# SiftScience/kafka-assigner

Hardware: NVIDIA H100
Metric: partition-replica assignments/sec (higher is better)
Workload: dtype int32

## Files before the change

### kafka_assigner_b200/csrc/kassign_common.cuh

```cuda
#pragma once
#include <cuda_runtime.h>
#include <stdint.h>

#define KA_MAX_SLOTS 8
#define KA_DEAD 0xFFFFu
#define KA_FULL 0xFFFFFFFFu

#define KA_E_RF_MISMATCH 1
#define KA_E_RF_NOT_POSITIVE 2
#define KA_E_RF_GT_BROKERS 3
#define KA_E_UNASSIGNABLE 4
#define KA_E_HASH_INDEX 5

enum { KA_LUT_SMEM = 0, KA_LUT_GLOBAL = 1, KA_LUT_BSEARCH = 2 };

struct KaBrokers {
    int N, lut_mode, lut_off, blob_bytes, min_id;
    uint32_t range;
    const uint16_t* blob;
    const uint16_t* glut;
    const int32_t* broker_id;
};

struct KaStageOut {
    unsigned char* rec;
    uint16_t* perm;
    int32_t* ntl;
    uint32_t* lend;
    int4* tstatus;
    unsigned* err_topic;
};

struct KaCandidate {
    KaBrokers br;
    KaStageOut out;
    int32_t* ctr8;
    const int32_t* loff;
    uint32_t pos0;
    int t0, T;
    uint32_t row0, Q;
    int desired_rf;
};

__device__ __forceinline__ uint32_t ka_lookup(int id, const uint16_t* lut, const KaBrokers& br) {
    if (br.lut_mode == KA_LUT_SMEM) {
        uint32_t off = (uint32_t)id - (uint32_t)br.min_id;
        return off < br.range ? (uint32_t)lut[off] : KA_DEAD;
    } else if (br.lut_mode == KA_LUT_GLOBAL) {
        uint32_t off = (uint32_t)id - (uint32_t)br.min_id;
        return off < br.range ? (uint32_t)__ldg(&br.glut[off]) : KA_DEAD;
    } else {
        int lo = 0, hi = br.N - 1;
        while (lo <= hi) {
            int mid = (lo + hi) >> 1;
            int v = __ldg(&br.broker_id[mid]);
            if (v == id) return (uint32_t)mid;
            if (v < id) lo = mid + 1; else hi = mid - 1;
        }
        return KA_DEAD;
    }
}



__device__ __forceinline__ uint32_t ka_smem_u32(const void* p) { return (uint32_t)__cvta_generic_to_shared(p); }

__device__ __forceinline__ void ka_mbar_init(uint64_t* bar, uint32_t count) {
    asm volatile("mbarrier.init.shared::cta.b64 [%0], %1;" ::"r"(ka_smem_u32(bar)), "r"(count));
}
__device__ __forceinline__ void ka_fence_mbar_init() { asm volatile("fence.mbarrier_init.release.cluster;" ::: "memory"); }
__device__ __forceinline__ void ka_fence_proxy_async() { asm volatile("fence.proxy.async.shared::cta;" ::: "memory"); }
__device__ __forceinline__ void ka_mbar_expect_tx(uint64_t* bar, uint32_t bytes) {
    asm volatile("mbarrier.arrive.expect_tx.shared::cta.b64 _, [%0], %1;" ::"r"(ka_smem_u32(bar)), "r"(bytes) : "memory");
}
__device__ __forceinline__ void ka_mbar_wait(uint64_t* bar, uint32_t parity) {
    asm volatile(
        "{\n"
        ".reg .pred p;\n"
        "WAIT_LOOP:\n"
        "mbarrier.try_wait.parity.shared::cta.b64 p, [%0], %1;\n"
        "@p bra WAIT_DONE;\n"
        "bra WAIT_LOOP;\n"
        "WAIT_DONE:\n"
        "}\n" ::"r"(ka_smem_u32(bar)),
        "r"(parity)
        : "memory");
}
__device__ __forceinline__ void ka_tma_bulk_g2s(void* dst_smem, const void* src_gmem, uint32_t bytes, uint64_t* bar) {
    asm volatile("cp.async.bulk.shared::cluster.global.mbarrier::complete_tx::bytes [%0], [%1], %2, [%3];" ::"r"(
                     ka_smem_u32(dst_smem)),
                 "l"(src_gmem), "r"(bytes), "r"(ka_smem_u32(bar))
                 : "memory");
}

__device__ __forceinline__ int4 ka_ldg_stream_v4(const int4* p) {
    int4 r;
    asm volatile("ld.global.nc.L1::no_allocate.v4.s32 {%0,%1,%2,%3}, [%4];" : "=r"(r.x), "=r"(r.y), "=r"(r.z), "=r"(r.w) : "l"(p));
    return r;
}

__device__ __forceinline__ uint32_t ka_lanemask_lt() {
    uint32_t m;
    asm("mov.u32 %0, %%lanemask_lt;" : "=r"(m));
    return m;
}

__device__ __forceinline__ uint32_t ka_rot_bits(uint32_t habs) {
    return ((habs % 2u) << 4) | ((habs % 3u) << 5) | ((habs % 4u) << 7) | ((habs % 5u) << 9) | ((habs % 6u) << 12) |
           ((habs % 7u) << 15) | ((habs % 8u) << 18);
}
template <int RS>
__device__ __forceinline__ int ka_rot_of(uint32_t meta, int k) {
    int s = 0;
    if (k == 2) s = (meta >> 4) & 1u;
    if (k == 3) s = (meta >> 5) & 3u;
    if (k == 4) s = (meta >> 7) & 3u;
    if (RS > 4) {
        if (k == 5) s = (meta >> 9) & 7u;
        if (k == 6) s = (meta >> 12) & 7u;
        if (k == 7) s = (meta >> 15) & 7u;
        if (k == 8) s = (meta >> 18) & 7u;
    }
    return s;
}
```

### kafka_assigner_b200/csrc/kassign_order.cuh

```cuda
#pragma once
#include "kassign_common.cuh"

__global__ void __launch_bounds__(1024) ka_level_scan_kernel(const int32_t* __restrict__ ntl, int T, int32_t* __restrict__ loff) {
    __shared__ int wsum[32];
    __shared__ int carry;
    const int lane = threadIdx.x & 31, warp = threadIdx.x >> 5;
    if (threadIdx.x == 0) carry = 0;
    __syncthreads();
    for (int t0 = 0; t0 < T; t0 += 1024) {
        const int t = t0 + threadIdx.x;
        const int v = t < T ? ntl[t] : 0;
        int x = v;
#pragma unroll
        for (int o = 1; o < 32; o <<= 1) {
            const int y = __shfl_up_sync(KA_FULL, x, o);
            if (lane >= o) x += y;
        }
        if (lane == 31) wsum[warp] = x;
        __syncthreads();
        if (warp == 0) {
            int w = wsum[lane];
#pragma unroll
            for (int o = 1; o < 32; o <<= 1) {
                const int y = __shfl_up_sync(KA_FULL, w, o);
                if (lane >= o) w += y;
            }
            wsum[lane] = w;
        }
        __syncthreads();
        const int base = carry + (warp > 0 ? wsum[warp - 1] : 0);
        if (t < T) loff[t] = base + x - v;
        __syncthreads();
        if (threadIdx.x == 1023) carry = base + x;
        __syncthreads();
    }
    if (threadIdx.x == 0) loff[T] = carry;
}

__global__ void __launch_bounds__(256) ka_level_fill_kernel(const int32_t* __restrict__ ntl, const int32_t* __restrict__ loff,
                                                            const uint32_t* __restrict__ lend, const int64_t* __restrict__ part_off, int P,
                                                            int T, int U, int64_t rows, uint32_t* __restrict__ lvl_end) {
    const int lane = threadIdx.x & 31;
    const int u = (blockIdx.x * blockDim.x + threadIdx.x) >> 5;
    if (u >= U) return;
    const int k = u / T, t = u - k * T;
    const int64_t g0 = (int64_t)k * rows + (part_off ? part_off[t] : (int64_t)t * P);
    const int d = ntl[u], o = loff[u];
    for (int l = lane; l < d; l += 32) lvl_end[o + l] = (uint32_t)g0 + lend[g0 + l];
}

struct KaOrderParams {
    uint32_t Q;
    int N;
    int S;
    const void* rec;
    uint32_t uniform_width;
    const uint32_t* chunk_end;
    const int32_t* chunk_lo_ptr;
    const int32_t* chunk_hi_ptr;
    uint32_t pos_base;
    int32_t* ctr8;
    const int32_t* broker_id;
    int32_t* out;
    int32_t* out_len;
    int ring_log2;
    const KaCandidate* cand;
    int cand_t0, cand_t1;
};

#define KA_RING_STAGES 8

__device__ __forceinline__ void ka_mbar_arrive(uint64_t* bar) {
    asm volatile("mbarrier.arrive.shared::cta.b64 _, [%0];" ::"r"(ka_smem_u32(bar)) : "memory");
}
__device__ __forceinline__ void ka_named_bar_sync(uint32_t id, uint32_t nthreads) {
    asm volatile("bar.sync %0, %1;" ::"r"(id), "r"(nthreads) : "memory");
}

template <bool GCTR> struct KaCtr;
template <> struct KaCtr<false> {
    typedef uint32_t H;
    template <int CW> static __device__ __forceinline__ H row(uint32_t sbase, int32_t*, uint32_t a) { return sbase + (CW == 4 ? a : a * 2u); }
    static __device__ __forceinline__ int4 ld4(H h, int off) {
        int4 v;
        asm volatile("ld.volatile.shared.v4.s32 {%0,%1,%2,%3}, [%4];" : "=r"(v.x), "=r"(v.y), "=r"(v.z), "=r"(v.w) : "r"(h + off));
        return v;
    }
    static __device__ __forceinline__ void st(H h, int off, int v) { asm volatile("st.volatile.shared.s32 [%0], %1;" ::"r"(h + off), "r"(v) : "memory"); }
    static __device__ __forceinline__ H col(uint32_t sbase, int32_t*, uint32_t a, int) { return sbase + a; }
    static __device__ __forceinline__ int ld1(H h) {
        int v;
        asm volatile("ld.volatile.shared.s32 %0, [%1];" : "=r"(v) : "r"(h));
        return v;
    }
    static __device__ __forceinline__ void st1(H h, int v) { asm volatile("st.volatile.shared.s32 [%0], %1;" ::"r"(h), "r"(v) : "memory"); }
};
template <> struct KaCtr<true> {
    typedef char* H;
    template <int CW> static __device__ __forceinline__ H row(uint32_t, int32_t* g, uint32_t a) { return reinterpret_cast<char*>(g) + (size_t)a * 2u; }
    static __device__ __forceinline__ int4 ld4(H h, int off) {
        int4 v;
        asm volatile("ld.volatile.global.v4.s32 {%0,%1,%2,%3}, [%4];" : "=r"(v.x), "=r"(v.y), "=r"(v.z), "=r"(v.w) : "l"(h + off));
        return v;
    }
    static __device__ __forceinline__ void st(H h, int off, int v) { asm volatile("st.volatile.global.s32 [%0], %1;" ::"l"(h + off), "r"(v) : "memory"); }
    static __device__ __forceinline__ H col(uint32_t, int32_t* g, uint32_t a, int slot) { return reinterpret_cast<char*>(g) + (size_t)a * 8u + slot * 4; }
    static __device__ __forceinline__ int ld1(H h) {
        int v;
        asm volatile("ld.volatile.global.s32 %0, [%1];" : "=r"(v) : "l"(h));
        return v;
    }
    static __device__ __forceinline__ void st1(H h, int v) { asm volatile("st.volatile.global.s32 [%0], %1;" ::"l"(h), "r"(v) : "memory"); }
};

template <int RS>
__device__ __forceinline__ void ka_order_generic(const int (&c)[RS][RS], int len, uint32_t meta, int (&perm)[RS]) {
    uint32_t remmask = (1u << len) - 1u;
#pragma unroll
    for (int r = 0; r < RS; ++r) {
        if (r < len) {
            const int k = len - r;
            const int s = ka_rot_of<RS>(meta, k);
            long long best = 0x7FFFFFFFFFFFFFFFLL;
            int bpos = 0;
#pragma unroll
            for (int pos = 0; pos < RS; ++pos) {
                if ((remmask >> pos) & 1u) {
                    int j = __popc(remmask & ((1u << pos) - 1u)) + s;
                    if (j >= k) j -= k;
                    const long long key = (long long)c[pos][r] * 8 + j;
                    if (key < best) { best = key; bpos = pos; }
                }
            }
            perm[r] = bpos;
            remmask &= ~(1u << bpos);
        }
    }
}

template <int KIND, bool GCTR, int MAXNT, bool SINGLE, bool WARP1, bool FULL, bool CAND = false>
__global__ void __launch_bounds__(MAXNT, 1) ka_order_levels_kernel(const KaOrderParams p) {
    constexpr int RS = KIND <= 1 ? 3 : KIND;
    constexpr int CW = KIND <= 1 ? 1 : (KIND == 4 ? 4 : 8);
    constexpr int RB = RS == 3 ? 16 : 32;
    constexpr int NS = KA_RING_STAGES;
    typedef KaCtr<GCTR> C;
    extern __shared__ __align__(128) unsigned char ka_osmem[];
    const uint32_t tid = threadIdx.x, lane = tid & 31;
    unsigned char* ring = ka_osmem;
    uint64_t* full = reinterpret_cast<uint64_t*>(ka_osmem + ((size_t)NS << p.ring_log2) * RB);
    volatile uint32_t* pin = reinterpret_cast<volatile uint32_t*>(full + 2 * NS);
    int* ctr = reinterpret_cast<int*>(ka_osmem + ((size_t)NS << p.ring_log2) * RB + 256);
    static_assert(!CAND || KIND <= 1, "batched solves order rows of <= 3 replicas");
    const KaCandidate* const cd = CAND ? p.cand + blockIdx.x : nullptr;
    if (CAND && (cd->br.N <= 0 || p.pos_base >= cd->Q)) return;
    if (tid == 0) {
        const void* const rec = CAND ? (const void*)(cd->out.rec + ((size_t)cd->row0 + p.pos_base) * RB) : p.rec;
        int32_t* const c8 = CAND ? cd->ctr8 : p.ctr8;
        pin[0] = CAND ? min(p.Q, cd->Q - p.pos_base) : p.Q;
        pin[1] = blockDim.x; pin[2] = (uint32_t)p.ring_log2; pin[3] = p.uniform_width;
        pin[4] = (uint32_t)reinterpret_cast<uintptr_t>(rec); pin[5] = (uint32_t)(reinterpret_cast<uintptr_t>(rec) >> 32);
        pin[6] = (uint32_t)reinterpret_cast<uintptr_t>(c8); pin[7] = (uint32_t)(reinterpret_cast<uintptr_t>(c8) >> 32);
        if (CAND) pin[8] = (uint32_t)cd->br.N;
    }
    __syncthreads();
    const uint32_t Q = pin[0], NT = pin[1];
    const int LG = (int)pin[2];
    const uint32_t w = pin[3];
    uint4* const orec = reinterpret_cast<uint4*>((uintptr_t)pin[4] | ((uintptr_t)pin[5] << 32));
    int32_t* const ctr8 = reinterpret_cast<int32_t*>((uintptr_t)pin[6] | ((uintptr_t)pin[7] << 32));
    const uint32_t G = 1u << LG;

    if (tid == 0) {
        for (int i = 0; i < NS; ++i) ka_mbar_init(&full[i], 1);
        ka_fence_mbar_init();
    }
    if (!GCTR)
        for (uint32_t i = tid; i < (uint32_t)(CAND ? (int)pin[8] : p.N) * CW; i += blockDim.x)
            ctr[i] = ctr8[(i / CW) * KA_MAX_SLOTS + (KIND <= 1 ? KIND : (int)(i % CW))];
    if (KIND <= 1 && tid == 0) {
        const int N = CAND ? (int)pin[8] : p.N;
        if (GCTR) ctr8[(size_t)N * KA_MAX_SLOTS + KIND] = 0x3FFFFFFF; else ctr[N] = 0x3FFFFFFF;
    }
    for (uint32_t i = tid; i < (uint32_t)NS * G * (RB / 16); i += blockDim.x) reinterpret_cast<uint4*>(ring)[i] = make_uint4(0, 0, 0, 0);
    ka_fence_proxy_async();
    __syncthreads();

    const uint32_t nstages_all = (Q + G - 1) >> LG;
    auto issue_stage = [&](uint32_t j) {
        const uint32_t slot = j & (NS - 1);
        const uint32_t bytes = min(G, Q - (j << LG)) * RB;
        ka_mbar_expect_tx(&full[slot], bytes);
        ka_tma_bulk_g2s(ring + (size_t)slot * G * RB, reinterpret_cast<const unsigned char*>(CAND ? (const void*)orec : p.rec) + (size_t)j * G * RB,
                        bytes, &full[slot]);
    };
    if (tid == 0)
        for (uint32_t j = 0; j < min(nstages_all, (uint32_t)NS); ++j) issue_stage(j);

    const uint32_t rmask = (uint32_t)NS * G - 1u;
    const uint32_t ring_s = ka_smem_u32(ring);
    uint32_t landed = 0;
    uint32_t released = 0;
    const int chunk_lo = w ? 0 : (CAND ? cd->loff[min(p.cand_t0, cd->T)] : *p.chunk_lo_ptr);
    const int nchunk = w ? 0 : (CAND ? cd->loff[min(p.cand_t1, cd->T)] : *p.chunk_hi_ptr) - chunk_lo;
    const uint32_t* const cend = p.chunk_end + chunk_lo;
    const uint32_t pos_base = CAND ? cd->pos0 + p.pos_base : p.pos_base;
    int wbase = 0;
    uint32_t wcur = Q, wnxt = Q;
    if (!w) {
        wcur = (int)lane < nchunk ? cend[lane] - pos_base : Q;
        wnxt = 32 + (int)lane < nchunk ? cend[32 + lane] - pos_base : Q;
    }
    uint32_t lvl_hi = w;
    int c = 0;
    auto next_end = [&](uint32_t cur_end) -> uint32_t {
        if (w) {
            if (cur_end == lvl_hi) lvl_hi += w;
            return min(min(cur_end + NT, lvl_hi), Q);
        }
        ++c;
        if (c >= nchunk) return Q;
        if (c >= wbase + 32) {
            wcur = wnxt;
            wbase += 32;
            const int i = wbase + 32 + (int)lane;
            wnxt = i < nchunk ? cend[i] - pos_base : Q;
        }
        return __shfl_sync(KA_FULL, wcur, c - wbase);
    };
    auto read_rec = [&](uint32_t pos, uint4& a, uint4& b) {
        const uint32_t src = ring_s + (pos & rmask) * RB;
        asm volatile("ld.volatile.shared.v4.u32 {%0,%1,%2,%3}, [%4];" : "=r"(a.x), "=r"(a.y), "=r"(a.z), "=r"(a.w) : "r"(src));
        if (RS != 3) asm volatile("ld.volatile.shared.v4.u32 {%0,%1,%2,%3}, [%4];" : "=r"(b.x), "=r"(b.y), "=r"(b.z), "=r"(b.w) : "r"(src + 16));
    };
    auto cross = [&](uint32_t held_end, uint32_t xlast) {
        if (tid == 0 && ((released + 1u) << LG) <= held_end) {
            ka_fence_proxy_async();
            while (((released + 1u) << LG) <= held_end) {
                if (released + NS < nstages_all) issue_stage(released + NS);
                ++released;
            }
        }
        const uint32_t j = xlast >> LG;
        while (landed <= j) { ka_mbar_wait(&full[landed & (NS - 1)], (landed / NS) & 1u); ++landed; }
    };

    const uint32_t cbase = GCTR ? 0u : ka_smem_u32(ctr);
    uint32_t start = 0, end = w ? min(min(NT, w), Q) : (nchunk > 0 ? __shfl_sync(KA_FULL, wcur, 0) : Q);
    uint32_t limit = 0;
    auto cross_to = [&](uint32_t held_end, uint32_t nend) {
        cross(held_end, nend - 1u);
        limit = landed << LG;
    };
    uint4 ra0 = make_uint4(0, 0, 0, 0), ra1 = ra0, rb0 = ra0, rb1 = ra0;
    cross_to(0, end);
    read_rec(start + tid, ra0, ra1);

#define KA_SLOT0_CORE(RC, ACTIVE, POS)                                                                                          \
            const uint32_t a0 = RC.x, a1 = RC.y, a2 = RC.z, f = RC.w;                                                           \
            const int x0 = C::ld1(C::col(cbase, ctr8, a0, 0)), x1 = C::ld1(C::col(cbase, ctr8, a1, 0)), x2 = C::ld1(C::col(cbase, ctr8, a2, 0));
#define KA_SLOT0_DECIDE(ACTIVE, POS)                                                                                            \
                      \
            const bool L10 = x1 < x0;                                                                                       \
            const int m01 = min(x0, x1);                                                                                    \
            const bool is2 = x2 < m01;                                                                                      \
            const uint32_t oA = is2 ? a2 : (L10 ? a1 : a0);                                                                 \
            const int vA = min(m01, x2);                                                                                    \
                                                               \
            const uint32_t op = is2 ? a0 : (L10 ? a0 : a1), oq = is2 ? a1 : a2;                                             \
            const uint32_t fz = f & 0x83u;                                                                                  \
            const uint32_t fo = is2 ? (fz | (f & 4u)) : (L10 ? (fz | ((f >> 1) & 4u)) : (fz | ((f >> 2) & 4u)));            \
            if (ACTIVE) {                                                                                                       \
                C::st1(C::col(cbase, ctr8, oA, 0), vA + 1);                          \
                asm volatile("st.global.v4.u32 [%0], {%1,%2,%3,%4};" ::"l"(orec + (POS)), "r"(op), "r"(oq), "r"(fo), "r"(oA) : "memory"); \
            }
#define KA_SLOT1_CORE(RC, ACTIVE, POS)                                                                                          \
            const uint32_t op = RC.x, oq = RC.y, f = RC.z, oA = RC.w;                                                           \
            const int yp = C::ld1(C::col(cbase, ctr8, op, 1)), yq = C::ld1(C::col(cbase, ctr8, oq, 1));
#define KA_SLOT1_DECIDE(ACTIVE, POS)                                                                                            \
            const bool pickq = yq < yp + (int)((f >> 2) & 1u);                                                                  \
            const uint32_t o1 = pickq ? oq : op, o2 = pickq ? op : oq;                                                          \
            if (ACTIVE) {                                                                                                       \
                C::st1(C::col(cbase, ctr8, o1, 1), (pickq ? yq : yp) + 1);           \
                                                           \
                asm volatile("st.global.v4.u32 [%0], {%1,%2,%3,%4};" ::"l"(orec + (POS)), "r"(oA), "r"(o1), "r"(o2), "r"(f) : "memory"); \
            }
    if (KIND <= 1 && WARP1) {
        const uint32_t lmle = ka_lanemask_lt() | (1u << lane);
        for (uint32_t wstart = 0; wstart < Q;) {
            const uint32_t pos = wstart + tid;
            const uint32_t f = KIND == 0 ? ra0.w : ra0.z;
            const uint32_t bal = __ballot_sync(KA_FULL, pos < Q && (f & 0x80u)) | 1u;
            const int ngrp = __popc(bal);
            const uint32_t take = 32u;
            const bool active = pos < Q;
            const int grp = __popc(bal & lmle) - 1;
            const uint32_t nstart = wstart + take, need = min(nstart + 32u, Q);
            if (__builtin_expect(need > limit, 0)) cross_to(nstart, need);
            read_rec(nstart + tid, rb0, rb1);
            if (KIND == 0) {
                const uint32_t a0 = ra0.x, a1 = ra0.y, a2 = ra0.z;
                bool is1 = false, is2 = false;
                for (int g = 0; g < ngrp; ++g) {
                    if (grp == g && active) {
                        const int x0 = C::ld1(C::col(cbase, ctr8, a0, 0)), x1 = C::ld1(C::col(cbase, ctr8, a1, 0)), x2 = C::ld1(C::col(cbase, ctr8, a2, 0));
                        const bool L10 = x1 < x0, L20 = x2 < x0, L21 = x2 < x1;
                        is2 = L10 ? L21 : L20;
                        is1 = L10 && !L21;
                        C::st1(C::col(cbase, ctr8, is2 ? a2 : (is1 ? a1 : a0), 0), (is2 ? x2 : (is1 ? x1 : x0)) + 1);
                    }
                    __syncwarp();
                }
                const bool is0 = !(is1 || is2);
                const uint32_t oA = is2 ? a2 : (is1 ? a1 : a0), op = is0 ? a1 : a0, oq = is2 ? a1 : a2;
                const uint32_t esh = is2 ? f : (is1 ? f >> 1 : f >> 2);
                if (active) asm volatile("st.global.v4.u32 [%0], {%1,%2,%3,%4};" ::"l"(orec + pos), "r"(op), "r"(oq), "r"((f & 0x83u) | (esh & 4u)), "r"(oA) : "memory");
            } else {
                const uint32_t op = ra0.x, oq = ra0.y, oA = ra0.w;
                bool pickq = false;
                for (int g = 0; g < ngrp; ++g) {
                    if (grp == g && active) {
                        const int yp = C::ld1(C::col(cbase, ctr8, op, 1)), yq = C::ld1(C::col(cbase, ctr8, oq, 1));
                        pickq = yq < yp + (int)((f >> 2) & 1u);
                        C::st1(C::col(cbase, ctr8, pickq ? oq : op, 1), (pickq ? yq : yp) + 1);
                    }
                    __syncwarp();
                }
                if (active) asm volatile("st.global.v4.u32 [%0], {%1,%2,%3,%4};" ::"l"(orec + pos), "r"(oA), "r"(pickq ? oq : op), "r"(pickq ? op : oq), "r"(f) : "memory");
            }
            ra0 = rb0;
            wstart = nstart;
        }
    } else if (KIND <= 1 && SINGLE) {
        const uint32_t nchunks = Q / w, nstages = (Q + G - 1) >> LG;
        const uint32_t w16 = w * RB, rmask16 = (uint32_t)NS * G * RB - 1u;
        const bool act = FULL || tid < w;
        uint32_t roff = (tid * RB) & rmask16;
        uint32_t pos = tid, k = 0;
#define KA_SINGLE_BODY(RC, RN)                                                                                                  \
        {                                                                                                                       \
            if (KIND == 0) {                                                                                                    \
                KA_SLOT0_CORE(RC, act, pos)                                                                                     \
                roff = (roff + w16) & rmask16;                                                                                  \
                asm volatile("ld.volatile.shared.v4.u32 {%0,%1,%2,%3}, [%4];" : "=r"(RN.x), "=r"(RN.y), "=r"(RN.z), "=r"(RN.w) : "r"(ring_s + roff)); \
                KA_SLOT0_DECIDE(act, pos)                                                                                       \
            } else {                                                                                                            \
                KA_SLOT1_CORE(RC, act, pos)                                                                                     \
                roff = (roff + w16) & rmask16;                                                                                  \
                asm volatile("ld.volatile.shared.v4.u32 {%0,%1,%2,%3}, [%4];" : "=r"(RN.x), "=r"(RN.y), "=r"(RN.z), "=r"(RN.w) : "r"(ring_s + roff)); \
                KA_SLOT1_DECIDE(act, pos)                                                                                       \
            }                                                                                                                   \
            if (WARP1) __syncwarp(); else __syncthreads();                                                   \
            pos += w;                                                                                                           \
        }
        const uint32_t cps = G / w, rps = G - cps * w;
        uint32_t lim_chunks = 0, lim_rem = 0;
        for (uint32_t sdone = 0; sdone < landed; ++sdone) {
            lim_chunks += cps; lim_rem += rps;
            if (lim_rem >= w) { lim_rem -= w; ++lim_chunks; }
        }
        while (k < nchunks) {
            while (landed < nstages && lim_chunks < k + 2) {
                if (tid == 0 && ((released + 1u) << LG) <= (k + 1) * w) {
                    ka_fence_proxy_async();
                    while (((released + 1u) << LG) <= (k + 1) * w) {
                        if (released + NS < nstages_all) issue_stage(released + NS);
                        ++released;
                    }
                }
                ka_mbar_wait(&full[landed & (NS - 1)], (landed / NS) & 1u);
                ++landed;
                lim_chunks += cps; lim_rem += rps;
                if (lim_rem >= w) { lim_rem -= w; ++lim_chunks; }
            }
            const uint32_t n = landed >= nstages ? nchunks - k : min(nchunks, lim_chunks - 1u) - k;
            uint32_t i = 0;
            for (; i + 4 <= n; i += 4) {
                KA_SINGLE_BODY(ra0, rb0)
                KA_SINGLE_BODY(rb0, ra0)
                KA_SINGLE_BODY(ra0, rb0)
                KA_SINGLE_BODY(rb0, ra0)
            }
            for (; i < n; ++i) {
                KA_SINGLE_BODY(ra0, rb0)
                ra0 = rb0;
            }
            k += n;
        }
#undef KA_SINGLE_BODY
    } else if (KIND <= 1) {
#define KA_SLOT_BODY(RC, RN)                                                                                                    \
        {                                                                                                                       \
            const uint32_t pos = start + tid;                                                                                   \
            const bool active = pos < end;                                                                                      \
            const uint32_t nstart = end;                                                                                        \
            if (KIND == 0) {                                                                                                    \
                KA_SLOT0_CORE(RC, active, pos)                                                                                  \
                                \
                const uint32_t nend = next_end(end);                                                                            \
                if (__builtin_expect(nend > limit, 0)) cross_to(end, nend);                         \
                read_rec(nstart + tid, RN, rb1);                                                                                \
                KA_SLOT0_DECIDE(active, pos)                                                                                    \
                end = nend;                                                                                                     \
            } else {                                                                                                            \
                KA_SLOT1_CORE(RC, active, pos)                                                                                  \
                const uint32_t nend = next_end(end);                                                                            \
                if (__builtin_expect(nend > limit, 0)) cross_to(end, nend);                                                     \
                read_rec(nstart + tid, RN, rb1);                                                                                \
                KA_SLOT1_DECIDE(active, pos)                                                                                    \
                end = nend;                                                                                                     \
            }                                                                                                                   \
                                   \
            if (WARP1) __syncwarp(); else __syncthreads();                                                             \
            start = nstart;                                                                                                     \
        }
        while (true) {
            KA_SLOT_BODY(ra0, rb0)
            if (start >= Q) break;
            KA_SLOT_BODY(rb0, ra0)
            if (start >= Q) break;
        }
#undef KA_SLOT_BODY
    } else {
        while (start < Q) {
            const uint32_t pos = start + tid;
            const bool active = pos < end;
            uint4 nb0, nb1;
            (void)pos;
            const uint32_t meta = active ? ra1.x : 0u;
            const uint32_t orow = ra1.y;
            const int len = (int)(meta & 15u);
            uint32_t av[RS];
            av[0] = (ra0.x & 0xFFFFu) << 4; av[1] = (ra0.x >> 16) << 4; av[2] = (ra0.y & 0xFFFFu) << 4; av[3] = (ra0.y >> 16) << 4;
            if (RS == 8) {
                av[4] = (ra0.z & 0xFFFFu) << 4; av[5] = (ra0.z >> 16) << 4; av[6] = (ra0.w & 0xFFFFu) << 4; av[7] = (ra0.w >> 16) << 4;
            }
            int cv[RS][RS];
#pragma unroll
            for (int i = 0; i < RS; ++i) {
                if (i < len) {
                    const typename C::H h = C::template row<CW>(cbase, ctr8, av[i]);
#pragma unroll
                    for (int v = 0; v < RS; v += 4) {
                        const int4 rw = C::ld4(h, v * 4);
                        cv[i][v] = rw.x; cv[i][v + 1] = rw.y; cv[i][v + 2] = rw.z; cv[i][v + 3] = rw.w;
                    }
                } else {
#pragma unroll
                    for (int v = 0; v < RS; ++v) cv[i][v] = 0;
                }
            }
            const uint32_t nstart = end;
            const uint32_t nend = next_end(end);
            if (nend > limit) cross_to(end, nend);
            read_rec(nstart + tid, nb0, nb1);
            int perm[RS];
#pragma unroll
            for (int i = 0; i < RS; ++i) perm[i] = i;
            if (len > 0) ka_order_generic<RS>(cv, len, meta, perm);
#pragma unroll
            for (int r = 0; r < RS; ++r) {
                if (r < len) {
                    uint32_t ba = 0;
                    int cc = 0;
#pragma unroll
                    for (int q = 0; q < RS; ++q)
                        if (perm[r] == q) { ba = av[q]; cc = cv[q][r]; }
                    C::st(C::template row<CW>(cbase, ctr8, ba), r * 4, cc + 1);
                    if (r < p.S) p.out[(size_t)orow * p.S + r] = __ldg(&p.broker_id[ba >> 4]);
                } else if (active && r < p.S) {
                    p.out[(size_t)orow * p.S + r] = -1;
                }
            }
            if (active && p.out_len) p.out_len[orow] = len;
            if (NT == 32) __syncwarp(); else __syncthreads();
            start = nstart; end = nend;
            ra0 = nb0; ra1 = nb1;
        }
    }

    if (!GCTR) {
        if (NT == 32) __syncwarp(); else __syncthreads();
        for (uint32_t i = tid; i < (uint32_t)(CAND ? (int)pin[8] : p.N) * CW; i += NT) ctr8[(i / CW) * KA_MAX_SLOTS + (KIND <= 1 ? KIND : (int)(i % CW))] = ctr[i];
    }
}

__device__ __forceinline__ void ka_emit3(const uint4* __restrict__ rec, const uint16_t* __restrict__ perm,
                                         const int64_t* __restrict__ part_off, int T, int P, const int32_t* __restrict__ broker_id,
                                         uint32_t Q, int S, int32_t* __restrict__ out, int32_t* __restrict__ out_len,
                                         int32_t* __restrict__ ctr8, uint32_t base = 0) {
    const uint32_t pos = blockIdx.x * blockDim.x + threadIdx.x;
    if (pos >= Q) return;
    const uint4 r = rec[pos];
    const int len = (int)(r.w & 3u);
    uint32_t row = pos;
    if (perm) {
        int64_t g0;
        if (part_off) {
            int lo = 0, hi = T;
            while (hi - lo > 1) {
                const int mid = (lo + hi) >> 1;
                if (part_off[mid] <= (int64_t)(base + pos)) lo = mid; else hi = mid;
            }
            g0 = part_off[lo] - base;
        } else {
            g0 = (int64_t)(pos / (uint32_t)P) * P;
        }
        row = (uint32_t)g0 + perm[pos];
    }
    int32_t* o = out + (size_t)row * S;
    o[0] = len > 0 ? __ldg(broker_id + (r.x >> 2)) : -1;
    if (S > 1) o[1] = len > 1 ? __ldg(broker_id + (r.y >> 2)) : -1;
    if (S > 2) o[2] = len > 2 ? __ldg(broker_id + (r.z >> 2)) : -1;
    if (out_len) out_len[row] = len;
    if (len > 2) atomicAdd(ctr8 + (size_t)(r.z >> 2) * KA_MAX_SLOTS + 2, 1);
}

__global__ void __launch_bounds__(256) ka_emit3_kernel(const uint4* __restrict__ rec, const uint16_t* __restrict__ perm,
                                                       const int64_t* __restrict__ part_off, int T, int P,
                                                       const int32_t* __restrict__ broker_id, uint32_t Q, int S, int32_t* __restrict__ out,
                                                       int32_t* __restrict__ out_len, int32_t* __restrict__ ctr8) {
    ka_emit3(rec, perm, part_off, T, P, broker_id, Q, S, out, out_len, ctr8);
}

template <bool RAGGED = false>
__global__ void __launch_bounds__(256) ka_emit3_candidates_kernel(const KaCandidate* __restrict__ cand, uint32_t r0, int T, int P,
                                                                  const int64_t* __restrict__ part_off, uint32_t Q, int S,
                                                                  int64_t cand_rows, int32_t* __restrict__ out,
                                                                  int32_t* __restrict__ out_len) {
    const KaCandidate& c = cand[blockIdx.y];
    if (c.br.N <= 0 || r0 >= c.Q) return;
    const uint32_t base = c.row0 + r0;
    const int64_t row0 = (int64_t)blockIdx.y * cand_rows + base;
    ka_emit3(reinterpret_cast<const uint4*>(c.out.rec) + base, c.out.perm ? c.out.perm + base : nullptr, RAGGED ? part_off + c.t0 : nullptr,
             RAGGED ? c.T : T, P, c.br.broker_id, min(Q, c.Q - r0), S, out + row0 * S, out_len ? out_len + row0 : nullptr, c.ctr8, base);
}
```

Measured before the change: 2.886 billion.

## Encode slot choices as flag bits instead of rewriting full 16-byte records

Slot 0 and slot 1 passes no longer store the whole reordered uint4 record. They write only the flags word, with two bits for the winner index and one bit for the slot-1 pick. Readers rebuild the reordered view through ka_slot1_view and ka_rec3_list, and the emit kernel decodes the final broker order from these bits. This cuts per-record store traffic from 16 bytes to 4 in each slot pass, at the cost of extra select logic when decoding.

```diff
diff --git a/kafka_assigner_b200/csrc/kassign_common.cuh b/kafka_assigner_b200/csrc/kassign_common.cuh
--- a/kafka_assigner_b200/csrc/kassign_common.cuh
+++ b/kafka_assigner_b200/csrc/kassign_common.cuh
@@ -61,6 +61,20 @@
     }
 }
 
+__host__ __device__ __forceinline__ uint32_t ka_f_w0(uint32_t f, uint32_t w0) { return f | (w0 << 8); }
+__host__ __device__ __forceinline__ uint32_t ka_f_w1(uint32_t f) { return f | (1u << 10); }
+
+__device__ __forceinline__ void ka_slot1_view(uint4& r) {
+    const uint32_t f = r.w, w0 = (f >> 8) & 3u;
+    r = make_uint4(w0 == 0 ? r.y : r.x, w0 == 2 ? r.y : r.z, f, (f >> (4u - w0)) & 1u);
+}
+
+__device__ __forceinline__ uint3 ka_rec3_list(uint4 r) {
+    const uint32_t w0 = (r.w >> 8) & 3u;
+    const uint32_t o0 = w0 == 0 ? r.x : (w0 == 1 ? r.y : r.z), op = w0 == 0 ? r.y : r.x, oq = w0 == 2 ? r.y : r.z;
+    const bool pickq = (r.w >> 10) & 1u;
+    return make_uint3(o0, pickq ? oq : op, pickq ? op : oq);
+}
 
 
 __device__ __forceinline__ uint32_t ka_smem_u32(const void* p) { return (uint32_t)__cvta_generic_to_shared(p); }
diff --git a/kafka_assigner_b200/csrc/kassign_order.cuh b/kafka_assigner_b200/csrc/kassign_order.cuh
--- a/kafka_assigner_b200/csrc/kassign_order.cuh
+++ b/kafka_assigner_b200/csrc/kassign_order.cuh
@@ -255,35 +255,32 @@
     uint4 ra0 = make_uint4(0, 0, 0, 0), ra1 = ra0, rb0 = ra0, rb1 = ra0;
     cross_to(0, end);
     read_rec(start + tid, ra0, ra1);
+    if (KIND == 1) ka_slot1_view(ra0);
 
 #define KA_SLOT0_CORE(RC, ACTIVE, POS)                                                                                          \
             const uint32_t a0 = RC.x, a1 = RC.y, a2 = RC.z, f = RC.w;                                                           \
             const int x0 = C::ld1(C::col(cbase, ctr8, a0, 0)), x1 = C::ld1(C::col(cbase, ctr8, a1, 0)), x2 = C::ld1(C::col(cbase, ctr8, a2, 0));
 #define KA_SLOT0_DECIDE(ACTIVE, POS)                                                                                            \
-                      \
+                                      \
             const bool L10 = x1 < x0;                                                                                       \
             const int m01 = min(x0, x1);                                                                                    \
             const bool is2 = x2 < m01;                                                                                      \
             const uint32_t oA = is2 ? a2 : (L10 ? a1 : a0);                                                                 \
             const int vA = min(m01, x2);                                                                                    \
-                                                               \
-            const uint32_t op = is2 ? a0 : (L10 ? a0 : a1), oq = is2 ? a1 : a2;                                             \
-            const uint32_t fz = f & 0x83u;                                                                                  \
-            const uint32_t fo = is2 ? (fz | (f & 4u)) : (L10 ? (fz | ((f >> 1) & 4u)) : (fz | ((f >> 2) & 4u)));            \
+            const uint32_t fw = is2 ? ka_f_w0(f, 2) : (L10 ? ka_f_w0(f, 1) : f);                                            \
             if (ACTIVE) {                                                                                                       \
                 C::st1(C::col(cbase, ctr8, oA, 0), vA + 1);                          \
-                asm volatile("st.global.v4.u32 [%0], {%1,%2,%3,%4};" ::"l"(orec + (POS)), "r"(op), "r"(oq), "r"(fo), "r"(oA) : "memory"); \
+                asm volatile("st.global.u32 [%0], %1;" ::"l"(&orec[POS].w), "r"(fw) : "memory");                                \
             }
 #define KA_SLOT1_CORE(RC, ACTIVE, POS)                                                                                          \
-            const uint32_t op = RC.x, oq = RC.y, f = RC.z, oA = RC.w;                                                           \
+            const uint32_t op = RC.x, oq = RC.y, f = RC.z, e = RC.w;                                                            \
             const int yp = C::ld1(C::col(cbase, ctr8, op, 1)), yq = C::ld1(C::col(cbase, ctr8, oq, 1));
 #define KA_SLOT1_DECIDE(ACTIVE, POS)                                                                                            \
-            const bool pickq = yq < yp + (int)((f >> 2) & 1u);                                                                  \
-            const uint32_t o1 = pickq ? oq : op, o2 = pickq ? op : oq;                                                          \
+            const bool pickq = yq < yp + (int)e;                                                                                \
+            const uint32_t fw = pickq ? ka_f_w1(f) : f;                                                                         \
             if (ACTIVE) {                                                                                                       \
-                C::st1(C::col(cbase, ctr8, o1, 1), (pickq ? yq : yp) + 1);           \
-                                                           \
-                asm volatile("st.global.v4.u32 [%0], {%1,%2,%3,%4};" ::"l"(orec + (POS)), "r"(oA), "r"(o1), "r"(o2), "r"(f) : "memory"); \
+                C::st1(C::col(cbase, ctr8, pickq ? oq : op, 1), (pickq ? yq : yp) + 1);    \
+                asm volatile("st.global.u32 [%0], %1;" ::"l"(&orec[POS].w), "r"(fw) : "memory");                                \
             }
     if (KIND <= 1 && WARP1) {
         const uint32_t lmle = ka_lanemask_lt() | (1u << lane);
@@ -311,22 +308,20 @@
                     }
                     __syncwarp();
                 }
-                const bool is0 = !(is1 || is2);
-                const uint32_t oA = is2 ? a2 : (is1 ? a1 : a0), op = is0 ? a1 : a0, oq = is2 ? a1 : a2;
-                const uint32_t esh = is2 ? f : (is1 ? f >> 1 : f >> 2);
-                if (active) asm volatile("st.global.v4.u32 [%0], {%1,%2,%3,%4};" ::"l"(orec + pos), "r"(op), "r"(oq), "r"((f & 0x83u) | (esh & 4u)), "r"(oA) : "memory");
+                if (active) asm volatile("st.global.u32 [%0], %1;" ::"l"(&orec[pos].w), "r"(ka_f_w0(f, is2 ? 2u : (is1 ? 1u : 0u))) : "memory");
             } else {
-                const uint32_t op = ra0.x, oq = ra0.y, oA = ra0.w;
+                const uint32_t op = ra0.x, oq = ra0.y, e = ra0.w;
                 bool pickq = false;
                 for (int g = 0; g < ngrp; ++g) {
                     if (grp == g && active) {
                         const int yp = C::ld1(C::col(cbase, ctr8, op, 1)), yq = C::ld1(C::col(cbase, ctr8, oq, 1));
-                        pickq = yq < yp + (int)((f >> 2) & 1u);
+                        pickq = yq < yp + (int)e;
                         C::st1(C::col(cbase, ctr8, pickq ? oq : op, 1), (pickq ? yq : yp) + 1);
                     }
                     __syncwarp();
                 }
-                if (active) asm volatile("st.global.v4.u32 [%0], {%1,%2,%3,%4};" ::"l"(orec + pos), "r"(oA), "r"(pickq ? oq : op), "r"(pickq ? op : oq), "r"(f) : "memory");
+                if (active) asm volatile("st.global.u32 [%0], %1;" ::"l"(&orec[pos].w), "r"(pickq ? ka_f_w1(f) : f) : "memory");
+                ka_slot1_view(rb0);
             }
             ra0 = rb0;
             wstart = nstart;
@@ -349,6 +344,7 @@
                 roff = (roff + w16) & rmask16;                                                                                  \
                 asm volatile("ld.volatile.shared.v4.u32 {%0,%1,%2,%3}, [%4];" : "=r"(RN.x), "=r"(RN.y), "=r"(RN.z), "=r"(RN.w) : "r"(ring_s + roff)); \
                 KA_SLOT1_DECIDE(act, pos)                                                                                       \
+                ka_slot1_view(RN);                                                                                              \
             }                                                                                                                   \
             if (WARP1) __syncwarp(); else __syncthreads();                                                   \
             pos += w;                                                                                                           \
@@ -408,6 +404,7 @@
                 if (__builtin_expect(nend > limit, 0)) cross_to(end, nend);                                                     \
                 read_rec(nstart + tid, RN, rb1);                                                                                \
                 KA_SLOT1_DECIDE(active, pos)                                                                                    \
+                ka_slot1_view(RN);                                                                                              \
                 end = nend;                                                                                                     \
             }                                                                                                                   \
                                    \
@@ -492,6 +489,7 @@
     const uint32_t pos = blockIdx.x * blockDim.x + threadIdx.x;
     if (pos >= Q) return;
     const uint4 r = rec[pos];
+    const uint3 o = ka_rec3_list(r);
     const int len = (int)(r.w & 3u);
     uint32_t row = pos;
     if (perm) {
@@ -508,12 +506,12 @@
         }
         row = (uint32_t)g0 + perm[pos];
     }
-    int32_t* o = out + (size_t)row * S;
-    o[0] = len > 0 ? __ldg(broker_id + (r.x >> 2)) : -1;
-    if (S > 1) o[1] = len > 1 ? __ldg(broker_id + (r.y >> 2)) : -1;
-    if (S > 2) o[2] = len > 2 ? __ldg(broker_id + (r.z >> 2)) : -1;
+    int32_t* orow = out + (size_t)row * S;
+    orow[0] = len > 0 ? __ldg(broker_id + (o.x >> 2)) : -1;
+    if (S > 1) orow[1] = len > 1 ? __ldg(broker_id + (o.y >> 2)) : -1;
+    if (S > 2) orow[2] = len > 2 ? __ldg(broker_id + (o.z >> 2)) : -1;
     if (out_len) out_len[row] = len;
-    if (len > 2) atomicAdd(ctr8 + (size_t)(r.z >> 2) * KA_MAX_SLOTS + 2, 1);
+    if (len > 2) atomicAdd(ctr8 + (size_t)(o.z >> 2) * KA_MAX_SLOTS + 2, 1);
 }
 
 __global__ void __launch_bounds__(256) ka_emit3_kernel(const uint4* __restrict__ rec, const uint16_t* __restrict__ perm,
```

Result: faster. 2.961 billion (median of 6 runs) (+2.6%).
